# wcy199705/DfFintheWild

Measured on AMD Instinct MI355X. Metric: focal-stacks/sec (10x3x256x256), higher is better.
Workload: dtype bf16x3 (split-bf16 MFMA operands hi+lo, fp32 accumulate, fp32-accurate); 1 GPU; DFF_net forward, 10-slice 3x256x256 focal stacks, batch 32 per GPU (BASELINE.json config 3), dense focus_dists, synthetic weights seed 0; batch_per_gpu=32, global_batch=32, slices=10, height=256, width=256, parallelism=single GPU, precision=bf16x3, input=float32 (B,3,N,H,W), the reference's tensor contract

## Files before the change

### dffinthewild_amd/csrc/dffw_srd_roll.hip

```cpp
#include <algorithm>
#include <cstdio>
#include <cstdlib>
#include <type_traits>

#include "dffw_device.h"
#include "dffw_persist.h"
#include "dffw_srd_roll.h"

namespace dffw {

using SrdRow = KernelRow<SrdArgs>;

template <int PREC, bool POOL, int ABL = 0>
__global__ __launch_bounds__(256) __attribute__((amdgpu_waves_per_eu(3))) void srd_roll_kernel(const SrdArgs a, const float *__restrict__ w3g, const float *__restrict__ w1g) {
    constexpr int PARTS = Fmt<PREC>::PARTS;
    constexpr bool F16 = (PREC == P_FP16);
    constexpr int C = 8, TY = 8, TX = 16, NWAVES = 4;
    constexpr int XY = TY + 4, XX = TX + 4, XPIX = XY * XX;
    constexpr int TYT = TY + 2, TXT = TX + 2, TPIX = TYT * TXT;
    constexpr int PIXB = C * 2;
    constexpr int NPIECE = (XPIX + 63) / 64;
    constexpr int PLANEB = NPIECE * 1024;
    constexpr int SLOTB = PARTS * PLANEB;
    constexpr int RX = 4;
    constexpr int NP = PARTS * NPIECE, PPW = (NP + NWAVES - 1) / NWAVES;
    static_assert(NP % PPW == 0, "every wave issues PPW pieces or none (counted vmcnt waits)");
    constexpr int TPLANEB = (TPIX * PIXB + 15) / 16 * 16;
    constexpr int FPLANEB = TY * TX * PIXB;
    constexpr int FSLOTB = PARTS * FPLANEB;
    constexpr int X_OFF = 0, T_OFF = RX * SLOTB, F_OFF = T_OFF + PARTS * TPLANEB;
    __shared__ __attribute__((aligned(1024))) unsigned char smem[F_OFF + 3 * FSLOTB];

    const int tid = threadIdx.x, lane = tid & 63, wave = tid >> 6;
    const int g = lane >> 4, r = lane & 15;
    const unsigned lds0 = (unsigned)(uintptr_t)(__attribute__((address_space(3))) unsigned char *)smem;
    typedef unsigned u32x2 __attribute__((ext_vector_type(2)));
    auto lds_store8 = [&](unsigned byte_off, uint32_t v0, uint32_t v1) {
        const u32x2 d = {v0, v1};
        asm volatile("ds_write_b64 %0, %1" ::"v"(lds0 + byte_off), "v"(d) : "memory");
    };
    auto lds_store16 = [&](unsigned byte_off, f32x4 v) { asm volatile("ds_write_b128 %0, %1" ::"v"(lds0 + byte_off), "v"(v) : "memory"); };

    const UnitRange ur = persistent_range(a.total_tiles);
    const int ufirst = ur.first, uend = ur.end, wgs_per_xcd = ur.step;
    if (ufirst >= uend) return;
    struct Unit {
        int b, gy0, gx0;
    };
    auto decode = [&](int u) {
        Unit c;
        const int txi = u % a.tiles_x;
        const int tt = u / a.tiles_x;
        c.b = tt / a.tiles_y;
        c.gy0 = (tt % a.tiles_y) * TY;
        c.gx0 = txi * TX;
        return c;
    };

    const int rec = PARTS * C;
    const int slice_elems = a.H * a.W * rec;
    const uint16_t *fsrc[PPW];
    bool fok[PPW];
    int fu = ufirst, fq = 0;
    auto setup_fill = [&]() {
        const Unit c = decode(fu);
#pragma unroll
        for (int k = 0; k < PPW; ++k) {
            const int p = wave * PPW + k;
            const int part = p / NPIECE, i = p % NPIECE;
            const int pix = i * 64 + lane;
            const int fy = pix / XX, sx = pix - fy * XX;
            const int fx = sx < XX / 2 ? 2 * sx : 2 * (sx - XX / 2) + 1;
            const int iy = c.gy0 - 2 + fy, ix = c.gx0 - 2 + fx;
            fok[k] = p < NP && pix < XPIX && (unsigned)iy < (unsigned)a.H && (unsigned)ix < (unsigned)a.W;
            fsrc[k] = a.x + (int64_t)c.b * a.N * slice_elems + (int64_t)(iy * a.W + ix) * rec + part * C;
        }
    };
    setup_fill();
    int fslot = 0;
    auto issue_next = [&]() {
        const bool zin = fu < uend;
        unsigned char *slot = smem + X_OFF + fslot * SLOTB;
        const int64_t zo = (int64_t)fq * slice_elems;
#pragma unroll
        for (int k = 0; k < PPW; ++k) {
            const int p = wave * PPW + k;
            if (p >= NP) break;
            const int part = p / NPIECE, i = p % NPIECE;
            const uint16_t *src = (zin && fok[k]) ? fsrc[k] + zo : a.zero;
            __builtin_amdgcn_global_load_lds((const __attribute__((address_space(1))) void *)src,
                                             (__attribute__((address_space(3))) void *)(slot + part * PLANEB + i * 1024), 16, 0, 0);
        }
        fslot = (fslot + 1 == RX) ? 0 : fslot + 1;
        if (++fq == a.N && fu < uend) {
            fq = 0;
            fu += wgs_per_xcd;
            if (fu < uend) setup_fill();
        }
    };

    constexpr int TA = 2;
    const int nA = wave < 2 ? 2 : 1;
    constexpr int APAIRS = TYT * (TXT / 2);
    int pa[TA], ta_y[TA], ta_x[TA], ta_st[TA];
    bool ta_ok[TA];
#pragma unroll
    for (int j = 0; j < TA; ++j) {
        const int tile = j == 0 ? wave : 4 + wave;
        int pi = tile * 16 + r;
        ta_ok[j] = pi < APAIRS;
        if (pi >= APAIRS) pi = APAIRS - 1;
        const int row = pi / (TXT / 2), pc = pi - row * (TXT / 2);
        ta_y[j] = row;
        ta_x[j] = 2 * pc + (g >> 1);
        pa[j] = (row * XX + ((g & 1) ? XX / 2 : 0) + pc + (g >> 1)) * PIXB;
        ta_st[j] = T_OFF + (row * TXT + ((g >> 1) ? TXT / 2 : 0) + pc) * PIXB + (g & 1) * 8;
    }
    const int pb_pi = wave * 16 + r, pb_y = pb_pi / (TX / 2), pb_pc = pb_pi % (TX / 2), pb_x = 2 * pb_pc + (g >> 1);
    const int pbo = (pb_y * TXT + ((g & 1) ? TXT / 2 : 0) + pb_pc + (g >> 1)) * PIXB;
    const int pb_res = ((pb_y + 2) * XX + (((pb_x + 2) & 1) ? XX / 2 : 0) + ((pb_x + 2) >> 1)) * PIXB + (g & 1) * 8;
    const int pb_f = (pb_y * TX + (g >> 1) * (TX / 2) + pb_pc) * PIXB;
    short8 w3f[2][PARTS], w1f[PARTS];
#pragma unroll
    for (int k = 0; k < 2; ++k)
#pragma unroll
        for (int pt = 0; pt < PARTS; ++pt) w3f[k][pt] = reinterpret_cast<const short8 *>(a.w3f)[(k * PARTS + pt) * 64 + lane];
#pragma unroll
    for (int pt = 0; pt < PARTS; ++pt) w1f[pt] = reinterpret_cast<const short8 *>(a.w1f)[pt * 64 + lane];
    short8 w0[3][PARTS], w2[3][PARTS];
#pragma unroll
    for (int k = 0; k < 3; ++k)
#pragma unroll
        for (int pt = 0; pt < PARTS; ++pt) {
            w0[k][pt] = reinterpret_cast<const short8 *>(a.w0)[(k * PARTS + pt) * 64 + lane];
            w2[k][pt] = reinterpret_cast<const short8 *>(a.w2)[(k * PARTS + pt) * 64 + lane];
        }
    const f32x4 b0 = *reinterpret_cast<const f32x4 *>(a.b0 + (g & 1) * 4);
    const f32x4 b2 = *reinterpret_cast<const f32x4 *>(a.b2 + (g & 1) * 4);
    auto tile_mma = [&](unsigned base, auto rowB_c, auto loB_c, const short8 (&wf)[3][PARTS], f32x4 acc) {
        constexpr int rowB = decltype(rowB_c)::value, loB = decltype(loB_c)::value;
        short8 xh[3], xl[3];
#define DFFW_SRD_READ(k)                                                                                                                  \
    asm volatile("ds_read_b128 %0, %1 offset:%2" : "=v"(xh[k]) : "v"(base), "n"(k * rowB));                                               \
    if constexpr (PARTS == 2) asm volatile("ds_read_b128 %0, %1 offset:%2" : "=v"(xl[k]) : "v"(base), "n"(k * rowB + loB));               \
    else xl[k] = short8{0, 0, 0, 0, 0, 0, 0, 0};
        DFFW_SRD_READ(0)
        DFFW_SRD_READ(1)
        DFFW_SRD_READ(2)
#undef DFFW_SRD_READ
#pragma unroll
        for (int k = 0; k < 3; ++k) {
            if (k == 0) asm volatile("s_waitcnt lgkmcnt(%2)" : "+v"(xh[0]), "+v"(xl[0]) : "n"(2 * PARTS));
            else if (k == 1) asm volatile("s_waitcnt lgkmcnt(%2)" : "+v"(xh[1]), "+v"(xl[1]) : "n"(PARTS));
            else asm volatile("s_waitcnt lgkmcnt(0)" : "+v"(xh[2]), "+v"(xl[2]));
            if constexpr (PARTS == 2) {
                acc = mma<F16>(wf[k][1], xh[k], acc);
                acc = mma<F16>(wf[k][0], xl[k], acc);
            }
            acc = mma<F16>(wf[k][0], xh[k], acc);
        }
        return acc;
    };

    constexpr int INFLIGHT = (RX - 2) * PPW;
#pragma unroll
    for (int q = 0; q < RX - 1; ++q) issue_next();
    __builtin_amdgcn_s_waitcnt(0x0F70);
    asm volatile("s_barrier" ::: "memory");

    int xslot = 0;
    f32x4 vq0 = f32x4{0.f, 0.f, 0.f, 0.f}, vq1 = vq0;
    typedef unsigned u32x4v __attribute__((ext_vector_type(4)));
    u32x4v fop = {0u, 0u, 0u, 0u};
#ifdef DFFW_TRACE_BUILD
    StepTrace trc(a.trace, wave, lane, NWAVES);
#else
    StepTrace trc(nullptr, wave, lane, NWAVES);
#endif
    for (int cu = ufirst; cu < uend; cu += wgs_per_xcd) {
        const Unit U = decode(cu);
        for (int s = 0; s <= a.N; ++s) {
            const bool produce = s < a.N;
            const unsigned fslot_off = F_OFF + (s % 3) * FSLOTB;
            trc.stamp(0);
            if (produce) {
                asm volatile("s_waitcnt vmcnt(%0)" ::"n"(INFLIGHT) : "memory");
                if constexpr (ABL & 16) asm volatile("s_waitcnt lgkmcnt(0)" ::: "memory"); else asm volatile("s_waitcnt lgkmcnt(0)\n\ts_barrier" ::: "memory");
            }
            trc.stamp(1);
            if (s == 0) {
                lds_store8(F_OFF + 2 * FSLOTB + pb_f + (g & 1) * 8, 0u, 0u);
                if constexpr (PARTS == 2) lds_store8(F_OFF + 2 * FSLOTB + FPLANEB + pb_f + (g & 1) * 8, 0u, 0u);
            }
            if (produce && !(ABL & 2)) {
                auto store_t = [&](int j, const f32x4 acc) {
                    const int iy = U.gy0 - 1 + ta_y[j], ix = U.gx0 - 1 + ta_x[j];
                    const bool inside = (unsigned)iy < (unsigned)a.H && (unsigned)ix < (unsigned)a.W;
                    if (ta_ok[j]) {
                        uint32_t h01, h23, l01, l23;
                        Fmt<PREC>::split2(relu_lim_bits(acc[0], inside ? 0x7f800000 : 0), relu_lim_bits(acc[1], inside ? 0x7f800000 : 0), h01, l01);
                        Fmt<PREC>::split2(relu_lim_bits(acc[2], inside ? 0x7f800000 : 0), relu_lim_bits(acc[3], inside ? 0x7f800000 : 0), h23, l23);
                        lds_store8(ta_st[j], h01, h23);
                        if constexpr (PARTS == 2) lds_store8(ta_st[j] + TPLANEB, l01, l23);
                    }
                };
                if (nA == 2) {
                    const unsigned ab0 = lds0 + X_OFF + xslot * SLOTB + pa[0], ab1 = lds0 + X_OFF + xslot * SLOTB + pa[1];
                    short8 ah[3], al[3];
#define DFFW_SRD_RDA(base, k)                                                                                                             \
    asm volatile("ds_read_b128 %0, %1 offset:%2" : "=v"(ah[k]) : "v"(base), "n"(k * XX * PIXB));                                           \
    if constexpr (PARTS == 2) asm volatile("ds_read_b128 %0, %1 offset:%2" : "=v"(al[k]) : "v"(base), "n"(k * XX * PIXB + PLANEB));
#define DFFW_SRD_MMA(k, W)                                 \
    if constexpr (PARTS == 2) {                            \
        acc = mma<F16>(w0[k][1], ah[k], acc);              \
        acc = mma<F16>(w0[k][0], al[k], acc);              \
    }                                                      \
    acc = mma<F16>(w0[k][0], ah[k], acc);
                    DFFW_SRD_RDA(ab0, 0)
                    DFFW_SRD_RDA(ab0, 1)
                    DFFW_SRD_RDA(ab0, 2)
                    f32x4 acc = b0;
                    if constexpr (PARTS == 2) asm volatile("s_waitcnt lgkmcnt(4)" : "+v"(ah[0]), "+v"(al[0])); else asm volatile("s_waitcnt lgkmcnt(2)" : "+v"(ah[0]));
                    DFFW_SRD_MMA(0, w0)
                    DFFW_SRD_RDA(ab1, 0)
                    if constexpr (PARTS == 2) asm volatile("s_waitcnt lgkmcnt(4)" : "+v"(ah[1]), "+v"(al[1])); else asm volatile("s_waitcnt lgkmcnt(2)" : "+v"(ah[1]));
                    DFFW_SRD_MMA(1, w0)
                    DFFW_SRD_RDA(ab1, 1)
                    if constexpr (PARTS == 2) asm volatile("s_waitcnt lgkmcnt(4)" : "+v"(ah[2]), "+v"(al[2])); else asm volatile("s_waitcnt lgkmcnt(2)" : "+v"(ah[2]));
                    DFFW_SRD_MMA(2, w0)
                    DFFW_SRD_RDA(ab1, 2)
                    store_t(0, acc);
                    acc = b0;
                    if constexpr (PARTS == 2) asm volatile("s_waitcnt lgkmcnt(4)" : "+v"(ah[0]), "+v"(al[0])); else asm volatile("s_waitcnt lgkmcnt(2)" : "+v"(ah[0]));
                    DFFW_SRD_MMA(0, w0)
                    if constexpr (PARTS == 2) asm volatile("s_waitcnt lgkmcnt(2)" : "+v"(ah[1]), "+v"(al[1])); else asm volatile("s_waitcnt lgkmcnt(1)" : "+v"(ah[1]));
                    DFFW_SRD_MMA(1, w0)
                    if constexpr (PARTS == 2) asm volatile("s_waitcnt lgkmcnt(0)" : "+v"(ah[2]), "+v"(al[2])); else asm volatile("s_waitcnt lgkmcnt(0)" : "+v"(ah[2]));
                    DFFW_SRD_MMA(2, w0)
#undef DFFW_SRD_RDA
#undef DFFW_SRD_MMA
                    store_t(1, acc);
                } else {
                    store_t(0, tile_mma(lds0 + X_OFF + xslot * SLOTB + pa[0], std::integral_constant<int, XX * PIXB>{}, std::integral_constant<int, PLANEB>{}, w0, b0));
                }
            }
            trc.stamp(2);
            if (produce) {
                if constexpr (ABL & 16) asm volatile("s_waitcnt lgkmcnt(0)" ::: "memory"); else asm volatile("s_waitcnt lgkmcnt(0)\n\ts_barrier" ::: "memory");
                trc.stamp(3);
                if constexpr (!(ABL & 4)) {
                    const f32x4 acc = tile_mma(lds0 + T_OFF + pbo, std::integral_constant<int, TXT * PIXB>{}, std::integral_constant<int, TPLANEB>{}, w2, b2);
                    const unsigned xp = lds0 + X_OFF + xslot * SLOTB + pb_res;
                    u32x2 xh, xl = {0u, 0u};
                    asm volatile("ds_read_b64 %0, %1" : "=v"(xh) : "v"(xp));
                    if constexpr (PARTS == 2) asm volatile("ds_read_b64 %0, %1 offset:%2" : "=v"(xl) : "v"(xp), "n"(PLANEB));
                    asm volatile("s_waitcnt lgkmcnt(0)" : "+v"(xh), "+v"(xl));
                    float r0, r1, r2, r3;
                    Fmt<PREC>::join2(xh[0], xl[0], r0, r1);
                    Fmt<PREC>::join2(xh[1], xl[1], r2, r3);
                    f32x4 v;
                    v[0] = relu_bits(acc[0] + r0);
                    v[1] = relu_bits(acc[1] + r1);
                    v[2] = relu_bits(acc[2] + r2);
                    v[3] = relu_bits(acc[3] + r3);
                    uint32_t fh01, fh23, fl01, fl23;
                    Fmt<PREC>::split2(v[0], v[1], fh01, fl01);
                    Fmt<PREC>::split2(v[2], v[3], fh23, fl23);
                    lds_store8(fslot_off + pb_f + (g & 1) * 8, fh01, fh23);
                    if constexpr (PARTS == 2) lds_store8(fslot_off + FPLANEB + pb_f + (g & 1) * 8, fl01, fl23);
                    fop = u32x4v{fh01, fh23, fl01, fl23};
                    vq1 = vq0;
                    vq0 = v;
                }
            } else {
                vq1 = vq0;
                fop = u32x4v{0u, 0u, 0u, 0u};
            }
            trc.stamp(4);
            if (s >= 1 && !(ABL & 1)) {
                const int z = s - 1;
                const unsigned sm = F_OFF + ((z + 2) % 3) * FSLOTB, sc = F_OFF + (z % 3) * FSLOTB;
                const unsigned ad0 = lds0 + ((g & 1) ? sc : sm) + pb_f;
                short8 fh0, fl0;
                asm volatile("ds_read_b128 %0, %1" : "=v"(fh0) : "v"(ad0));
                if constexpr (PARTS == 2) {
                    asm volatile("ds_read_b128 %0, %1 offset:%2" : "=v"(fl0) : "v"(ad0), "n"(FPLANEB));
                    asm volatile("s_waitcnt lgkmcnt(0)" : "+v"(fh0), "+v"(fl0));
                } else {
                    asm volatile("s_waitcnt lgkmcnt(0)" : "+v"(fh0));
                }
                const short8 f1op = __builtin_bit_cast(short8, fop);
                f32x4 at = f32x4{0.f, 0.f, 0.f, 0.f};
                if constexpr (PARTS == 2) {
                    at = mma<F16>(w3f[1][1], f1op, at);
                    at = mma<F16>(w3f[0][1], fh0, at);
                    at = mma<F16>(w3f[0][0], fl0, at);
                }
                at = mma<F16>(w3f[1][0], f1op, at);
                at = mma<F16>(w3f[0][0], fh0, at);
                uint32_t ah01, ah23, al01, al23;
                Fmt<PREC>::split2(relu_bits(at[0]), relu_bits(at[1]), ah01, al01);
                Fmt<PREC>::split2(relu_bits(at[2]), relu_bits(at[3]), ah23, al23);
                const u32x4v bq = {ah01, ah23, al01, al23};
                const short8 b2op = __builtin_bit_cast(short8, bq);
                f32x4 o = f32x4{0.f, 0.f, 0.f, 0.f};
                if constexpr (PARTS == 2) o = mma<F16>(w1f[1], b2op, o);
                o = mma<F16>(w1f[0], b2op, o);
                f32x4 v;
#pragma unroll
                for (int i = 0; i < 4; ++i) v[i] = vq1[i] + relu_bits(o[i]);
                uint32_t h01, h23, l01, l23;
                Fmt<PREC>::split2(v[0], v[1], h01, l01);
                Fmt<PREC>::split2(v[2], v[3], h23, l23);
                const int64_t pix = (((int64_t)U.b * a.N + z) * a.H + U.gy0 + pb_y) * a.W + U.gx0 + pb_x;
                if constexpr (POOL) {
                    float m[4];
                    Fmt<PREC>::join2(h01, l01, m[0], m[1]);
                    Fmt<PREC>::join2(h23, l23, m[2], m[3]);
                    uint32_t ph01, ph23, pl01, pl23;
#pragma unroll
                    for (int i = 0; i < 4; ++i) {
                        uint32_t mu = __float_as_uint(m[i]);
                        const auto sw = __builtin_amdgcn_permlane32_swap(mu, mu, false, false);
                        mu = max(mu, lane < 32 ? sw[1] : sw[0]);
                        mu = max(mu, (uint32_t)__builtin_amdgcn_mov_dpp((int)mu, 0x128, 0xF, 0xF, true));
                        m[i] = __uint_as_float(mu);
                    }
                    Fmt<PREC>::split2(m[0], m[1], ph01, pl01);
                    Fmt<PREC>::split2(m[2], m[3], ph23, pl23);
                    if constexpr (PARTS == 2) {
                        swap16(ph01, pl01);
                        swap16(ph23, pl23);
                    }
                    if (g < 2 && r < 8 && !(ABL & 32)) {
                        const int64_t pp = (((int64_t)U.b * a.N + z) * (a.H / 2) + (U.gy0 / 2 + wave)) * (a.W / 2) + U.gx0 / 2 + pb_pc;
                        if constexpr (PARTS == 2) *reinterpret_cast<uint4 *>(a.pooled + pp * rec + (g & 1) * C) = make_uint4(ph01, ph23, pl01, pl23);
                        else *reinterpret_cast<uint2 *>(a.pooled + pp * rec + (g & 1) * 4) = make_uint2(ph01, ph23);
                    }
                }
                if constexpr (PARTS == 2) {
                    swap16(h01, l01);
                    swap16(h23, l23);
                    if ((ABL & 32) == 0 || h01 == 0x12345u) *reinterpret_cast<uint4 *>(a.out + pix * rec + (g & 1) * C) = make_uint4(h01, h23, l01, l23);
                } else {
                    *reinterpret_cast<uint2 *>(a.out + pix * rec + (g & 1) * 4) = make_uint2(h01, h23);
                }
            }
            trc.stamp(5);
            if (produce) {
                if constexpr (ABL & 16) asm volatile("s_waitcnt lgkmcnt(0)" ::: "memory"); else asm volatile("s_waitcnt lgkmcnt(0)\n\ts_barrier" ::: "memory");
                trc.stamp(6);
                if constexpr (!(ABL & 8)) issue_next();
                xslot = (xslot + 1 == RX) ? 0 : xslot + 1;
            }
            trc.next();
        }
    }
    asm volatile("s_waitcnt vmcnt(0)" ::: "memory");
}

template <int PREC, bool POOL, int ABL = 0>
__global__ __launch_bounds__(256) __attribute__((amdgpu_waves_per_eu(2))) void srd_roll16_kernel(const SrdArgs a) {
    constexpr int PARTS = Fmt<PREC>::PARTS;
    constexpr bool F16 = (PREC == P_FP16);
    constexpr int C = 16, TY = 4, TX = 16, NWAVES = 4;
    constexpr int XY = TY + 4, XX = TX + 4, XPIX = XY * XX;
    constexpr int TYT = TY + 2, TXT = TX + 2, TPIX = TYT * TXT;
    constexpr int TXTP = 24;
    constexpr int PIXB = C * 2;
    constexpr int NPIECE = 6;
    static_assert(NPIECE * 32 >= XPIX, "plane holds the footprint");
    constexpr int PLANEB = NPIECE * 1024;
    constexpr int SLOTB = PARTS * PLANEB;
    constexpr int RX = 4;
    constexpr int NP = PARTS * NPIECE, PPW = (NP + NWAVES - 1) / NWAVES;
    static_assert(NP % PPW == 0, "every wave issues PPW pieces or none (counted vmcnt waits)");
    constexpr int TPLANEB = TYT * TXTP * PIXB;
    constexpr int FPLANEB = TY * TX * PIXB;
    constexpr int FSLOTB = PARTS * FPLANEB;
    constexpr int X_OFF = 0, T_OFF = RX * SLOTB, F_OFF = T_OFF + PARTS * TPLANEB;
    constexpr int NCH = 5;
    __shared__ __attribute__((aligned(1024))) unsigned char smem[F_OFF + 3 * FSLOTB];

    const int tid = threadIdx.x, lane = tid & 63, wave = tid >> 6;
    const int g = lane >> 4, r = lane & 15;
    const unsigned lds0 = (unsigned)(uintptr_t)(__attribute__((address_space(3))) unsigned char *)smem;
    typedef unsigned u32x2 __attribute__((ext_vector_type(2)));
    auto lds_store8 = [&](unsigned byte_off, uint32_t v0, uint32_t v1) {
        const u32x2 d = {v0, v1};
        asm volatile("ds_write_b64 %0, %1" ::"v"(lds0 + byte_off), "v"(d) : "memory");
    };
    auto lds_store16 = [&](unsigned byte_off, f32x4 v) { asm volatile("ds_write_b128 %0, %1" ::"v"(lds0 + byte_off), "v"(v) : "memory"); };

    const UnitRange ur = persistent_range(a.total_tiles);
    const int ufirst = ur.first, uend = ur.end, wgs_per_xcd = ur.step;
    if (ufirst >= uend) return;
    struct Unit {
        int b, gy0, gx0;
    };
    auto decode = [&](int u) {
        Unit c;
        const int txi = u % a.tiles_x;
        const int tt = u / a.tiles_x;
        c.b = tt / a.tiles_y;
        c.gy0 = (tt % a.tiles_y) * TY;
        c.gx0 = txi * TX;
        return c;
    };

    const int rec = PARTS * C;
    const int slice_elems = a.H * a.W * rec;
    const uint16_t *fsrc[PPW];
    bool fok[PPW];
    int fu = ufirst, fq = 0;
    auto setup_fill = [&]() {
        const Unit c = decode(fu);
#pragma unroll
        for (int k = 0; k < PPW; ++k) {
            const int p = wave * PPW + k;
            const int part = p / NPIECE, i = p % NPIECE;
            const int ci = i * 64 + lane, pix = ci >> 1, oct = ci & 1;
            const int fy = pix / XX, fx = pix - fy * XX;
            const int iy = c.gy0 - 2 + fy, ix = c.gx0 - 2 + fx;
            fok[k] = p < NP && pix < XPIX && (unsigned)iy < (unsigned)a.H && (unsigned)ix < (unsigned)a.W;
            fsrc[k] = a.x + (int64_t)c.b * a.N * slice_elems + (int64_t)(iy * a.W + ix) * rec + part * C + oct * 8;
        }
    };
    setup_fill();
    int fslot = 0;
    auto issue_next = [&]() {
        const bool zin = fu < uend;
        unsigned char *slot = smem + X_OFF + fslot * SLOTB;
        const int64_t zo = (int64_t)fq * slice_elems;
#pragma unroll
        for (int k = 0; k < PPW; ++k) {
            const int p = wave * PPW + k;
            if (p >= NP) break;
            const int part = p / NPIECE, i = p % NPIECE;
            const uint16_t *src = (zin && fok[k]) ? fsrc[k] + zo : a.zero;
            __builtin_amdgcn_global_load_lds((const __attribute__((address_space(1))) void *)src,
                                             (__attribute__((address_space(3))) void *)(slot + part * PLANEB + i * 1024), 16, 0, 0);
        }
        fslot = (fslot + 1 == RX) ? 0 : fslot + 1;
        if (++fq == a.N && fu < uend) {
            fq = 0;
            fu += wgs_per_xcd;
            if (fu < uend) setup_fill();
        }
    };

    constexpr int TA = 2;
    const int nA = wave < 3 ? 2 : 1;
    int pa[TA], ta_y[TA], ta_x[TA], ta_st[TA];
    bool ta_ok[TA];
#pragma unroll
    for (int j = 0; j < TA; ++j) {
        const int tile = j == 0 ? wave : 4 + wave;
        ta_ok[j] = tile < TYT || r < 2 * TYT;
        ta_y[j] = tile < TYT ? tile : (r < 2 * TYT ? r >> 1 : TYT - 1);
        ta_x[j] = tile < TYT ? r : TX + (r & 1);
        pa[j] = (ta_y[j] * XX + ta_x[j]) * PIXB + (g & 1) * 16;
        ta_st[j] = T_OFF + (ta_y[j] * TXTP + ta_x[j]) * PIXB + g * 8;
    }
    int tapA[NCH], tapB[NCH];
#pragma unroll
    for (int k = 0; k < NCH; ++k) {
        const int tap = 2 * k + (g >> 1);
        const int dy = tap < 9 ? tap / 3 : 0, dx = tap < 9 ? tap % 3 : 0;
        tapA[k] = (dy * XX + dx) * PIXB;
        tapB[k] = (dy * TXTP + dx) * PIXB;
    }
    const int pb_y = 2 * (wave >> 1) + (r >> 3), pb_x = 8 * (wave & 1) + (r & 7);
    const int pbo = (pb_y * TXTP + pb_x) * PIXB + (g & 1) * 16;
    const int pb_res = ((pb_y + 2) * XX + pb_x + 2) * PIXB + g * 8;
    const int pb_f = (pb_y * TX + pb_x) * PIXB;
    short8 w0[NCH][PARTS], w2[NCH][PARTS], w3f[2][PARTS], w1f[PARTS];
#pragma unroll
    for (int k = 0; k < NCH; ++k)
#pragma unroll
        for (int pt = 0; pt < PARTS; ++pt) {
            w0[k][pt] = reinterpret_cast<const short8 *>(a.w0)[(k * PARTS + pt) * 64 + lane];
            w2[k][pt] = reinterpret_cast<const short8 *>(a.w2)[(k * PARTS + pt) * 64 + lane];
        }
#pragma unroll
    for (int k = 0; k < 2; ++k)
#pragma unroll
        for (int pt = 0; pt < PARTS; ++pt) w3f[k][pt] = reinterpret_cast<const short8 *>(a.w3f)[(k * PARTS + pt) * 64 + lane];
#pragma unroll
    for (int pt = 0; pt < PARTS; ++pt) w1f[pt] = reinterpret_cast<const short8 *>(a.w1f)[pt * 64 + lane];
    const f32x4 b0 = *reinterpret_cast<const f32x4 *>(a.b0 + g * 4);
    const f32x4 b2 = *reinterpret_cast<const f32x4 *>(a.b2 + g * 4);
    auto tile_mma = [&](unsigned base, const int (&tapo)[NCH], auto loB_c, const short8 (&wf)[NCH][PARTS], f32x4 acc) {
        constexpr int loB = decltype(loB_c)::value;
        short8 xh[NCH], xl[NCH];
#pragma unroll
        for (int k = 0; k < NCH; ++k) {
            const unsigned ad = base + tapo[k];
            asm volatile("ds_read_b128 %0, %1" : "=v"(xh[k]) : "v"(ad));
            if constexpr (PARTS == 2) asm volatile("ds_read_b128 %0, %1 offset:%2" : "=v"(xl[k]) : "v"(ad), "n"(loB));
            else xl[k] = short8{0, 0, 0, 0, 0, 0, 0, 0};
        }
#pragma unroll
        for (int k = 0; k < NCH; ++k) {
            const int left = (NCH - 1 - k) * PARTS;
            if (left == 8) asm volatile("s_waitcnt lgkmcnt(8)" : "+v"(xh[k]), "+v"(xl[k]));
            else if (left == 6) asm volatile("s_waitcnt lgkmcnt(6)" : "+v"(xh[k]), "+v"(xl[k]));
            else if (left == 4) asm volatile("s_waitcnt lgkmcnt(4)" : "+v"(xh[k]), "+v"(xl[k]));
            else if (left == 3) asm volatile("s_waitcnt lgkmcnt(3)" : "+v"(xh[k]), "+v"(xl[k]));
            else if (left == 2) asm volatile("s_waitcnt lgkmcnt(2)" : "+v"(xh[k]), "+v"(xl[k]));
            else if (left == 1) asm volatile("s_waitcnt lgkmcnt(1)" : "+v"(xh[k]), "+v"(xl[k]));
            else asm volatile("s_waitcnt lgkmcnt(0)" : "+v"(xh[k]), "+v"(xl[k]));
            if constexpr (PARTS == 2) {
                acc = mma<F16>(wf[k][1], xh[k], acc);
                acc = mma<F16>(wf[k][0], xl[k], acc);
            }
            acc = mma<F16>(wf[k][0], xh[k], acc);
        }
        return acc;
    };

    auto tile_mma2 = [&](unsigned base0, unsigned base1, const int (&tapo)[NCH], auto loB_c, const short8 (&wf)[NCH][PARTS], f32x4 &acc0, f32x4 &acc1) {
        static_assert(PARTS == 2 || PARTS == 1, "");
        constexpr int NBUF = 3;
        short8 xh[NBUF][2], xl[NBUF][2];
        auto fetch = [&](int k) {
            const unsigned a0 = base0 + tapo[k], a1 = base1 + tapo[k];
            asm volatile("ds_read_b128 %0, %1" : "=v"(xh[k % NBUF][0]) : "v"(a0));
            if constexpr (PARTS == 2) asm volatile("ds_read_b128 %0, %1 offset:%2" : "=v"(xl[k % NBUF][0]) : "v"(a0), "n"(decltype(loB_c)::value));
            asm volatile("ds_read_b128 %0, %1" : "=v"(xh[k % NBUF][1]) : "v"(a1));
            if constexpr (PARTS == 2) asm volatile("ds_read_b128 %0, %1 offset:%2" : "=v"(xl[k % NBUF][1]) : "v"(a1), "n"(decltype(loB_c)::value));
        };
        fetch(0);
        fetch(1);
        fetch(2);
#pragma unroll
        for (int k = 0; k < NCH; ++k) {
            const int left = (NCH - 1 - k < 2 ? NCH - 1 - k : 2) * 2 * PARTS;
            auto &h0 = xh[k % NBUF][0], &h1 = xh[k % NBUF][1], &l0 = xl[k % NBUF][0], &l1 = xl[k % NBUF][1];
            if (left == 8) asm volatile("s_waitcnt lgkmcnt(8)" : "+v"(h0), "+v"(h1), "+v"(l0), "+v"(l1));
            else if (left == 4) asm volatile("s_waitcnt lgkmcnt(4)" : "+v"(h0), "+v"(h1), "+v"(l0), "+v"(l1));
            else if (left == 2) asm volatile("s_waitcnt lgkmcnt(2)" : "+v"(h0), "+v"(h1), "+v"(l0), "+v"(l1));
            else asm volatile("s_waitcnt lgkmcnt(0)" : "+v"(h0), "+v"(h1), "+v"(l0), "+v"(l1));
            if constexpr (PARTS == 1) {
                l0 = h0;
                l1 = h1;
            }
            if constexpr (PARTS == 2) {
                acc0 = mma<F16>(wf[k][1], h0, acc0);
                acc1 = mma<F16>(wf[k][1], h1, acc1);
                acc0 = mma<F16>(wf[k][0], l0, acc0);
                acc1 = mma<F16>(wf[k][0], l1, acc1);
            }
            acc0 = mma<F16>(wf[k][0], h0, acc0);
            acc1 = mma<F16>(wf[k][0], h1, acc1);
// ... 739 lines not shown
```

Baseline: 4136 stacks/s.

## Re-layout LDS x and t tiles to cut bank conflicts in residual conv

Changes the shared-memory layout of the staged input tile to a column-parity split with a 9-wide row stride and a folded tail region, and pads the intermediate t plane to a 24-pixel row stride with natural column order. Per-row read addresses are now precomputed per lane and passed to the MMA read helper, and the output pixel-to-lane mapping is permuted. The intent is to reduce LDS bank conflicts on the ds_read_b128 loads feeding the MFMA convolutions. In exchange it costs more address registers and more complex fill index math, which could increase register pressure.

```diff
diff --git a/dffinthewild_amd/csrc/dffw_srd_roll.hip b/dffinthewild_amd/csrc/dffw_srd_roll.hip
--- a/dffinthewild_amd/csrc/dffw_srd_roll.hip
+++ b/dffinthewild_amd/csrc/dffw_srd_roll.hip
@@ -17,7 +17,7 @@
     constexpr bool F16 = (PREC == P_FP16);
     constexpr int C = 8, TY = 8, TX = 16, NWAVES = 4;
     constexpr int XY = TY + 4, XX = TX + 4, XPIX = XY * XX;
-    constexpr int TYT = TY + 2, TXT = TX + 2, TPIX = TYT * TXT;
+    constexpr int TYT = TY + 2, TXT = TX + 2;
     constexpr int PIXB = C * 2;
     constexpr int NPIECE = (XPIX + 63) / 64;
     constexpr int PLANEB = NPIECE * 1024;
@@ -25,7 +25,9 @@
     constexpr int RX = 4;
     constexpr int NP = PARTS * NPIECE, PPW = (NP + NWAVES - 1) / NWAVES;
     static_assert(NP % PPW == 0, "every wave issues PPW pieces or none (counted vmcnt waits)");
-    constexpr int TPLANEB = (TPIX * PIXB + 15) / 16 * 16;
+    constexpr int XPL = 128, XH9 = 112, TXTP = 24;
+    static_assert(NPIECE * 64 == 2 * XPL && 9 * XY <= XH9 && XH9 + 16 <= XPL, "an x plane holds both column parities");
+    constexpr int TPLANEB = TYT * TXTP * PIXB;
     constexpr int FPLANEB = TY * TX * PIXB;
     constexpr int FSLOTB = PARTS * FPLANEB;
     constexpr int X_OFF = 0, T_OFF = RX * SLOTB, F_OFF = T_OFF + PARTS * TPLANEB;
@@ -68,11 +70,13 @@
         for (int k = 0; k < PPW; ++k) {
             const int p = wave * PPW + k;
             const int part = p / NPIECE, i = p % NPIECE;
-            const int pix = i * 64 + lane;
-            const int fy = pix / XX, sx = pix - fy * XX;
-            const int fx = sx < XX / 2 ? 2 * sx : 2 * (sx - XX / 2) + 1;
+            const int sl = i * 64 + lane, m = sl & (XPL - 1);
+            const int e9 = (9 * (m - XH9)) & 15;
+            const int fy = m < 9 * XY ? m / 9 : e9 - 1;
+            const int fx = (m < 9 * XY ? 2 * (m - 9 * fy) : XX - 2) + (sl >> 7);
+            const bool live = m < 9 * XY || (m >= XH9 && e9 >= 1 && e9 <= XY);
             const int iy = c.gy0 - 2 + fy, ix = c.gx0 - 2 + fx;
-            fok[k] = p < NP && pix < XPIX && (unsigned)iy < (unsigned)a.H && (unsigned)ix < (unsigned)a.W;
+            fok[k] = p < NP && live && (unsigned)iy < (unsigned)a.H && (unsigned)ix < (unsigned)a.W;
             fsrc[k] = a.x + (int64_t)c.b * a.N * slice_elems + (int64_t)(iy * a.W + ix) * rec + part * C;
         }
     };
@@ -99,27 +103,29 @@
         }
     };
 
+    auto xslot_of = [&](int y, int col) { return (col & 1) * XPL + ((col >> 1) < 9 ? 9 * y + (col >> 1) : XH9 + ((9 * (y + 1)) & 15)); };
     constexpr int TA = 2;
     const int nA = wave < 2 ? 2 : 1;
     constexpr int APAIRS = TYT * (TXT / 2);
-    int pa[TA], ta_y[TA], ta_x[TA], ta_st[TA];
+    int pa[TA][3], ta_y[TA], ta_x[TA], ta_st[TA];
     bool ta_ok[TA];
 #pragma unroll
     for (int j = 0; j < TA; ++j) {
         const int tile = j == 0 ? wave : 4 + wave;
         int pi = tile * 16 + r;
         ta_ok[j] = pi < APAIRS;
-        if (pi >= APAIRS) pi = APAIRS - 1;
+        if (pi >= APAIRS) pi -= 16;
         const int row = pi / (TXT / 2), pc = pi - row * (TXT / 2);
         ta_y[j] = row;
         ta_x[j] = 2 * pc + (g >> 1);
-        pa[j] = (row * XX + ((g & 1) ? XX / 2 : 0) + pc + (g >> 1)) * PIXB;
-        ta_st[j] = T_OFF + (row * TXT + ((g >> 1) ? TXT / 2 : 0) + pc) * PIXB + (g & 1) * 8;
+#pragma unroll
+        for (int k = 0; k < 3; ++k) pa[j][k] = xslot_of(row + k, 2 * pc + g) * PIXB;
+        ta_st[j] = T_OFF + (row * TXTP + ta_x[j]) * PIXB + (g & 1) * 8;
     }
-    const int pb_pi = wave * 16 + r, pb_y = pb_pi / (TX / 2), pb_pc = pb_pi % (TX / 2), pb_x = 2 * pb_pc + (g >> 1);
-    const int pbo = (pb_y * TXT + ((g & 1) ? TXT / 2 : 0) + pb_pc + (g >> 1)) * PIXB;
-    const int pb_res = ((pb_y + 2) * XX + (((pb_x + 2) & 1) ? XX / 2 : 0) + ((pb_x + 2) >> 1)) * PIXB + (g & 1) * 8;
-    const int pb_f = (pb_y * TX + (g >> 1) * (TX / 2) + pb_pc) * PIXB;
+    const int pb_rb = (r >> 3) ^ ((r >> 2) & 1), pb_y = 2 * wave + pb_rb, pb_pc = r & 7, pb_x = 2 * pb_pc + (g >> 1);
+    const int pbo = (pb_y * TXTP + 2 * pb_pc + g) * PIXB;
+    const int pb_res = xslot_of(pb_y + 2, pb_x + 2) * PIXB + (g & 1) * 8;
+    const int pb_f = (wave * 32 + (g >> 1) * 16 + pb_rb * 8 + pb_pc) * PIXB;
     short8 w3f[2][PARTS], w1f[PARTS];
 #pragma unroll
     for (int k = 0; k < 2; ++k)
@@ -137,12 +143,12 @@
         }
     const f32x4 b0 = *reinterpret_cast<const f32x4 *>(a.b0 + (g & 1) * 4);
     const f32x4 b2 = *reinterpret_cast<const f32x4 *>(a.b2 + (g & 1) * 4);
-    auto tile_mma = [&](unsigned base, auto rowB_c, auto loB_c, const short8 (&wf)[3][PARTS], f32x4 acc) {
+    auto tile_mma = [&](const unsigned (&base)[3], auto rowB_c, auto loB_c, const short8 (&wf)[3][PARTS], f32x4 acc) {
         constexpr int rowB = decltype(rowB_c)::value, loB = decltype(loB_c)::value;
         short8 xh[3], xl[3];
 #define DFFW_SRD_READ(k)                                                                                                                  \
-    asm volatile("ds_read_b128 %0, %1 offset:%2" : "=v"(xh[k]) : "v"(base), "n"(k * rowB));                                               \
-    if constexpr (PARTS == 2) asm volatile("ds_read_b128 %0, %1 offset:%2" : "=v"(xl[k]) : "v"(base), "n"(k * rowB + loB));               \
+    asm volatile("ds_read_b128 %0, %1 offset:%2" : "=v"(xh[k]) : "v"(base[k]), "n"(k * rowB));                                            \
+    if constexpr (PARTS == 2) asm volatile("ds_read_b128 %0, %1 offset:%2" : "=v"(xl[k]) : "v"(base[k]), "n"(k * rowB + loB));            \
     else xl[k] = short8{0, 0, 0, 0, 0, 0, 0, 0};
         DFFW_SRD_READ(0)
         DFFW_SRD_READ(1)
@@ -205,11 +211,12 @@
                     }
                 };
                 if (nA == 2) {
-                    const unsigned ab0 = lds0 + X_OFF + xslot * SLOTB + pa[0], ab1 = lds0 + X_OFF + xslot * SLOTB + pa[1];
+                    const unsigned xb = lds0 + X_OFF + xslot * SLOTB;
+                    const unsigned ab0[3] = {xb + pa[0][0], xb + pa[0][1], xb + pa[0][2]}, ab1[3] = {xb + pa[1][0], xb + pa[1][1], xb + pa[1][2]};
                     short8 ah[3], al[3];
 #define DFFW_SRD_RDA(base, k)                                                                                                             \
-    asm volatile("ds_read_b128 %0, %1 offset:%2" : "=v"(ah[k]) : "v"(base), "n"(k * XX * PIXB));                                           \
-    if constexpr (PARTS == 2) asm volatile("ds_read_b128 %0, %1 offset:%2" : "=v"(al[k]) : "v"(base), "n"(k * XX * PIXB + PLANEB));
+    asm volatile("ds_read_b128 %0, %1" : "=v"(ah[k]) : "v"(base[k]));                                                                     \
+    if constexpr (PARTS == 2) asm volatile("ds_read_b128 %0, %1 offset:%2" : "=v"(al[k]) : "v"(base[k]), "n"(PLANEB));
 #define DFFW_SRD_MMA(k, W)                                 \
     if constexpr (PARTS == 2) {                            \
         acc = mma<F16>(w0[k][1], ah[k], acc);              \
@@ -241,7 +248,9 @@
 #undef DFFW_SRD_MMA
                     store_t(1, acc);
                 } else {
-                    store_t(0, tile_mma(lds0 + X_OFF + xslot * SLOTB + pa[0], std::integral_constant<int, XX * PIXB>{}, std::integral_constant<int, PLANEB>{}, w0, b0));
+                    const unsigned xb = lds0 + X_OFF + xslot * SLOTB;
+                    const unsigned ab0[3] = {xb + pa[0][0], xb + pa[0][1], xb + pa[0][2]};
+                    store_t(0, tile_mma(ab0, std::integral_constant<int, 0>{}, std::integral_constant<int, PLANEB>{}, w0, b0));
                 }
             }
             trc.stamp(2);
@@ -249,7 +258,8 @@
                 if constexpr (ABL & 16) asm volatile("s_waitcnt lgkmcnt(0)" ::: "memory"); else asm volatile("s_waitcnt lgkmcnt(0)\n\ts_barrier" ::: "memory");
                 trc.stamp(3);
                 if constexpr (!(ABL & 4)) {
-                    const f32x4 acc = tile_mma(lds0 + T_OFF + pbo, std::integral_constant<int, TXT * PIXB>{}, std::integral_constant<int, TPLANEB>{}, w2, b2);
+                    const unsigned tb[3] = {lds0 + T_OFF + pbo, lds0 + T_OFF + pbo, lds0 + T_OFF + pbo};
+                    const f32x4 acc = tile_mma(tb, std::integral_constant<int, TXTP * PIXB>{}, std::integral_constant<int, TPLANEB>{}, w2, b2);
                     const unsigned xp = lds0 + X_OFF + xslot * SLOTB + pb_res;
                     u32x2 xh, xl = {0u, 0u};
                     asm volatile("ds_read_b64 %0, %1" : "=v"(xh) : "v"(xp));
```

Measured after the change: 4121 stacks/s. Within noise of the previous version (-0.4%).
